# Boese0601/MagicDance

Hardware: NVIDIA H100
Metric: denoise-steps/sec @512x512 50-step DDIM (higher is better)
Workload: dtype f16

## Files before the change

### magicdance_b200/csrc/attention.cu

```cuda
#include <stdlib.h>

#include <type_traits>

#include "common.cuh"

namespace mdb {

constexpr int kBQ = 128;

template <int D, int BKV, int STAGES>
struct AttnCfg {
  static constexpr int kDkChunks = (D + 63) / 64;
  static constexpr int kDV = (D + 15) / 16 * 16;
  static constexpr int kKSteps = kDV / 16;
  static constexpr int kQBytes = kDkChunks * kBQ * 128;
  static constexpr int kKBytes = kDkChunks * BKV * 128;
  static constexpr int kVBytes = kDV * 128;
  static constexpr int kStageBytes = kKBytes + kVBytes;
  static constexpr int kSmem = kQBytes + STAGES * kStageBytes + 1024;
  static_assert(BKV == 64, "one 128-byte swizzle row of keys per V^T tile");
  static_assert(kVBytes % 1024 == 0 && kKBytes % 1024 == 0, "stage tiles start on swizzle-atom boundaries");
};

struct AttnKParams {
  CUtensorMap tmQ, tmK0, tmV0, tmK1, tmV1;
  __half* out;
  long long ldo;
  int nq, n0, n1;
  int kv0_batches, kv1_batches;
  int bank_batches;
  float scale_log2;
};
struct AttnLseKParams : AttnKParams {
  float* lse;
};

template <int D, int BKV, int STAGES, int MINB, bool LSE = false>
__global__ void __launch_bounds__(kWsThreads, MINB)
    attn_wg_kernel(const __grid_constant__ std::conditional_t<LSE, AttnLseKParams, AttnKParams> p) {
  using C = AttnCfg<D, BKV, STAGES>;
  extern __shared__ uint8_t smem_raw[];
  __shared__ __align__(8) uint64_t q_bar;
  __shared__ __align__(8) uint64_t kv_full[STAGES], kv_empty[STAGES];

  uint8_t* sQ = align1024(smem_raw);
  uint8_t* sKV = sQ + C::kQBytes;

  const int warp = threadIdx.x >> 5;
  const int lane = threadIdx.x & 31;
  const int q0 = blockIdx.x * kBQ;
  const int head = blockIdx.y;
  const int b = blockIdx.z;
  const int t0 = (p.n0 + BKV - 1) / BKV;
  const int t1 = (b < p.bank_batches && p.n1 > 0) ? (p.n1 + BKV - 1) / BKV : 0;
  const int n_tiles = t0 + t1;

  pdl_launch_dependents();
  if (warp == kProducerWarp && lane == 0) {
    tma_prefetch_desc(&p.tmQ);
    tma_prefetch_desc(&p.tmK0);
    tma_prefetch_desc(&p.tmV0);
    mbar_init(&q_bar, 1);
    ring_init<STAGES>(kv_full, kv_empty, 1);
    fence_barrier_init();
  }
  __syncthreads();
  pdl_wait();

  if (warp == kProducerWarp) {
    if (lane == 0) {
      mbar_expect_tx(&q_bar, C::kQBytes);
      for (int dc = 0; dc < C::kDkChunks; ++dc)
        tma_load_3d(sQ + dc * (kBQ * 128), &p.tmQ, &q_bar, dc * 64, head, b * p.nq + q0);
      for (int j = 0; j < n_tiles; ++j) {
        const bool src1 = j >= t0;
        const int key0 = (src1 ? (j - t0) : j) * BKV;
        const CUtensorMap* tk = src1 ? &p.tmK1 : &p.tmK0;
        const CUtensorMap* tv = src1 ? &p.tmV1 : &p.tmV0;
        const int nsrc = src1 ? p.n1 : p.n0;
        const int kvb = src1 ? (p.kv1_batches > 1 ? b : 0) : (p.kv0_batches > 1 ? b : 0);
        const int s = ring_acquire<STAGES>(kv_empty, j);
        mbar_expect_tx(&kv_full[s], C::kStageBytes);
        uint8_t* sk = sKV + s * C::kStageBytes;
        uint8_t* sv = sk + C::kKBytes;
        for (int dc = 0; dc < C::kDkChunks; ++dc)
          tma_load_3d(sk + dc * (BKV * 128), tk, &kv_full[s], dc * 64, head, kvb * nsrc + key0);
        tma_load_3d(sv, tv, &kv_full[s], key0, kvb, head * D);
      }
    }
  } else {
    const int wg = warp >> 2;
    const uint32_t q_addr = smem_u32(sQ) + wg * (64 * 128);
    const int cq = 2 * (lane & 3);
    float o[C::kDV / 2];
#pragma unroll
    for (int i = 0; i < C::kDV / 2; ++i) o[i] = 0.f;
    float m_run[2] = {-INFINITY, -INFINITY};
    float l_run[2] = {0.f, 0.f};
    mbar_wait(&q_bar, 0);

    for (int j = 0; j < n_tiles; ++j) {
      const bool src1 = j >= t0;
      const int key0 = (src1 ? (j - t0) : j) * BKV;
      const int valid = min(BKV, (src1 ? p.n1 : p.n0) - key0);
      const int s = ring_wait_full<STAGES>(kv_full, j);
      const uint32_t k_addr = smem_u32(sKV + s * C::kStageBytes);
      const uint32_t v_addr = k_addr + C::kKBytes;

      float sc[BKV / 2];
      wgmma_fence();
#pragma unroll
      for (int ks = 0; ks < C::kKSteps; ++ks) {
        const int dc = ks >> 2, kk = ks & 3;
        const uint64_t da = wgmma_desc_k_sw128(q_addr + dc * (kBQ * 128)) + 2 * kk;
        const uint64_t db = wgmma_desc_k_sw128(k_addr + dc * (BKV * 128)) + 2 * kk;
        wgmma_ss<BKV>(sc, da, db, ks != 0 ? 1u : 0u);
      }
      wgmma_commit();
      wgmma_wait<0>();
      wgmma_fence_regs(sc);

      if (valid < BKV) {
#pragma unroll
        for (int i = 0; i < BKV / 2; ++i)
          if (8 * (i >> 2) + cq + (i & 1) >= valid) sc[i] = -INFINITY;
      }
      float mx[2] = {-INFINITY, -INFINITY};
#pragma unroll
      for (int i = 0; i < BKV / 2; ++i) mx[(i >> 1) & 1] = fmaxf(mx[(i >> 1) & 1], sc[i]);
      float alpha[2], neg_m[2];
#pragma unroll
      for (int h = 0; h < 2; ++h) {
        mx[h] = fmaxf(mx[h], __shfl_xor_sync(0xffffffffu, mx[h], 1));
        mx[h] = fmaxf(mx[h], __shfl_xor_sync(0xffffffffu, mx[h], 2));
        const float m_new = fmaxf(m_run[h], mx[h] * p.scale_log2);
        alpha[h] = ex2_approx(m_run[h] - m_new);
        m_run[h] = m_new;
        neg_m[h] = -m_new;
      }
      float ls[2] = {0.f, 0.f};
      uint32_t pa[BKV / 16][4];
#pragma unroll
      for (int i = 0; i < BKV / 2; i += 2) {
        const int h = (i >> 1) & 1;
        const float e0 = ex2_approx(fmaf(sc[i], p.scale_log2, neg_m[h]));
        const float e1 = ex2_approx(fmaf(sc[i + 1], p.scale_log2, neg_m[h]));
        ls[h] += e0 + e1;
        pa[i >> 3][(i >> 1) & 3] = pack_half2(e0, e1);
      }
#pragma unroll
      for (int h = 0; h < 2; ++h) l_run[h] = fmaf(l_run[h], alpha[h], ls[h]);
#pragma unroll
      for (int i = 0; i < C::kDV / 2; ++i) o[i] *= alpha[(i >> 1) & 1];

      wgmma_fence();
#pragma unroll
      for (int kk = 0; kk < BKV / 16; ++kk)
        wgmma_rs<C::kDV>(o, pa[kk], wgmma_desc_k_sw128(v_addr) + 2 * kk, 1u);
      wgmma_commit();
      wgmma_wait<0>();
      wgmma_fence_regs(o);
      mbar_arrive(&kv_empty[s]);
    }

    float inv_l[2], l_row[2];
#pragma unroll
    for (int h = 0; h < 2; ++h) {
      float l = l_run[h];
      l += __shfl_xor_sync(0xffffffffu, l, 1);
      l += __shfl_xor_sync(0xffffffffu, l, 2);
      inv_l[h] = 1.0f / l;
      l_row[h] = l;
    }
    const int r = wg * 64 + (warp & 3) * 16 + (lane >> 2);
    if constexpr (LSE) {
      if ((lane & 3) == 0) {
#pragma unroll
        for (int h = 0; h < 2; ++h) {
          const int q = q0 + r + 8 * h;
          if (q < p.nq)
            p.lse[(static_cast<long long>(b) * gridDim.y + head) * p.nq + q] =
                (m_run[h] + log2f(l_row[h])) * 0.6931471805599453f;
        }
      }
    }
#pragma unroll
    for (int h = 0; h < 2; ++h) {
      const int q = q0 + r + 8 * h;
      if (q < p.nq) {
        __half* op = p.out + (static_cast<long long>(b) * p.nq + q) * p.ldo + head * D + cq;
#pragma unroll
        for (int c8 = 0; c8 < D / 8; ++c8)
          *reinterpret_cast<uint32_t*>(op + 8 * c8) =
              pack_half2(o[4 * c8 + 2 * h] * inv_l[h], o[4 * c8 + 2 * h + 1] * inv_l[h]);
      }
    }
  }
}

static int g_attn40_2q_min_ctas = 512;
int get_attn_tuning() { return g_attn40_2q_min_ctas; }
void set_attn_tuning(int v) { g_attn40_2q_min_ctas = v; }

template <int D, int BKV, int STAGES, int MINB, bool LSE = false, typename P>
static int launch_attn(const P& kp, dim3 grid, cudaStream_t st) {
  using C = AttnCfg<D, BKV, STAGES>;
  static_assert(MINB == 1 || C::kSmem <= 113 * 1024, "two CTAs per SM must fit");
  constexpr auto kern = attn_wg_kernel<D, BKV, STAGES, MINB, LSE>;
  if (int rc = set_max_dyn_smem<kern>(C::kSmem)) return rc;
  MDB_CHECK_CUDA(launch_pdl(kern, grid, dim3(kWsThreads), C::kSmem, st, kp));
  count_launch();
  return MDB_OK;
}

template <int D, int BKV>
static int build_and_launch(const mdb_attn_desc* a, float* lse, cudaStream_t st) {
  constexpr int kDV = AttnCfg<D, BKV, 1>::kDV;
  AttnKParams kp;
  memset(&kp, 0, sizeof(kp));
  const int hd = a->heads * a->d;
  int rc;
  if ((rc = tmap_heads(&kp.tmQ, a->q, a->d, a->heads, (uint64_t)a->batch * a->nq, a->ldq, kBQ))) return rc;
  auto mk_kv = [&](const void* k, long long ldk, const void* vt, long long ldvt, int n, int nb, int ldvb,
                   CUtensorMap* tk, CUtensorMap* tv) -> int {
    int r = tmap_heads(tk, k, a->d, a->heads, (uint64_t)nb * n, ldk, BKV);
    if (r) return r;
    return tmap_vt(tv, vt, n, nb, ldvb, hd, ldvt, kDV);
  };
  if ((rc = mk_kv(a->k0, a->ldk0, a->vt0, a->ldvt0, a->n0, a->kv0_batches, a->ldv0_batch, &kp.tmK0, &kp.tmV0))) return rc;
  if (a->n1 > 0) {
    if ((rc = mk_kv(a->k1, a->ldk1, a->vt1, a->ldvt1, a->n1, a->kv1_batches, a->ldv1_batch, &kp.tmK1, &kp.tmV1)))
      return rc;
  }
  kp.out = static_cast<__half*>(a->out);
  kp.ldo = a->ldo;
  kp.nq = a->nq;
  kp.n0 = a->n0;
  kp.n1 = a->n1;
  kp.kv0_batches = a->kv0_batches;
  kp.kv1_batches = a->kv1_batches;
  kp.bank_batches = a->n1 > 0 ? a->bank_batches : 0;
  kp.scale_log2 = a->scale * 1.4426950408889634f;
  dim3 grid((a->nq + kBQ - 1) / kBQ, a->heads, a->batch);
  if (lse != nullptr) {
    AttnLseKParams lp;
    memset(&lp, 0, sizeof(lp));
    static_cast<AttnKParams&>(lp) = kp;
    lp.lse = lse;
    if constexpr (D == 40) {
      const long long ctas = (long long)grid.x * grid.y * grid.z;
      if (ctas >= (long long)g_attn40_2q_min_ctas) return launch_attn<D, BKV, 3, 2, true>(lp, grid, st);
    }
    return launch_attn<D, BKV, (D == 160 ? 2 : 4), 1, true>(lp, grid, st);
  }
  if constexpr (D == 40) {
    const long long ctas = (long long)grid.x * grid.y * grid.z;
    if (ctas >= (long long)g_attn40_2q_min_ctas) return launch_attn<D, BKV, 3, 2>(kp, grid, st);
  }
  return launch_attn<D, BKV, (D == 160 ? 2 : 4), 1>(kp, grid, st);
}

static int attention_entry(const mdb_attn_desc* a, float* lse, cudaStream_t st) {
  switch (a->d) {
    case 40:
      return build_and_launch<40, 64>(a, lse, st);
    case 80:
      return build_and_launch<80, 64>(a, lse, st);
    case 160:
      return build_and_launch<160, 64>(a, lse, st);
    default:
      set_error("mdb_attention_f16: head dim %d not supported (40, 80, 160)", a->d);
      return MDB_ERR_UNSUPPORTED;
  }
}

int attention_check_desc(const mdb_attn_desc* a) {
  MDB_REQUIRE(a != nullptr, "mdb_attention_f16: null descriptor");
  MDB_REQUIRE(a->q && a->k0 && a->vt0 && a->out, "mdb_attention_f16: null operand");
  MDB_REQUIRE(a->batch > 0 && a->heads > 0 && a->nq > 0 && a->n0 > 0 && a->n1 >= 0,
              "mdb_attention_f16: bad shape");
  MDB_REQUIRE(a->n1 == 0 || (a->k1 && a->vt1), "mdb_attention_f16: n1 > 0 needs k1/vt1");
  MDB_REQUIRE(a->kv0_batches == 1 || a->kv0_batches == a->batch, "mdb_attention_f16: kv0_batches must be 1 or batch");
  MDB_REQUIRE(a->n1 == 0 || a->kv1_batches == 1 || a->kv1_batches >= a->bank_batches,
              "mdb_attention_f16: kv1_batches must be 1 or cover bank_batches");
  MDB_REQUIRE(a->ldv0_batch >= a->n0 && a->ldv0_batch % 8 == 0, "mdb_attention_f16: ldv0_batch must be >= n0 and %% 8");
  MDB_REQUIRE(a->n1 == 0 || (a->ldv1_batch >= a->n1 && a->ldv1_batch % 8 == 0),
              "mdb_attention_f16: ldv1_batch must be >= n1 and %% 8");
  MDB_REQUIRE(a->ldo % 8 == 0 && (reinterpret_cast<uintptr_t>(a->out) & 15) == 0, "mdb_attention_f16: out alignment");
  return MDB_OK;
}

}

using namespace mdb;

extern "C" int mdb_attention_f16(const mdb_attn_desc* a, mdb_stream_t stream) {
  const int rc = attention_check_desc(a);
  if (rc) return rc;
  return attention_entry(a, nullptr, static_cast<cudaStream_t>(stream));
}

extern "C" int mdb_attention_lse_f16(const mdb_attn_desc* a, float* lse, mdb_stream_t stream) {
  const int rc = attention_check_desc(a);
  if (rc) return rc;
  MDB_REQUIRE(lse != nullptr, "mdb_attention_lse_f16: null lse");
  return attention_entry(a, lse, static_cast<cudaStream_t>(stream));
}
```

### magicdance_b200/csrc/common.cuh

```cuda
#pragma once

#include <cuda.h>
#include <cuda_fp16.h>
#include <cuda_runtime.h>
#include <cudaTypedefs.h>
#include <stdint.h>
#include <stdio.h>
#include <string.h>

#include "../../include/magicdance_b200.h"
#include "wgmma.cuh"

namespace mdb {

void set_error(const char* fmt, ...);

#define MDB_CHECK_CUDA(expr)                                                                     \
  do {                                                                                           \
    cudaError_t _e = (expr);                                                                     \
    if (_e != cudaSuccess) {                                                                     \
      mdb::set_error("%s:%d: %s failed: %s", __FILE__, __LINE__, #expr, cudaGetErrorString(_e)); \
      return MDB_ERR_CUDA;                                                                       \
    }                                                                                            \
  } while (0)

#define MDB_REQUIRE(cond, ...)      \
  do {                              \
    if (!(cond)) {                  \
      mdb::set_error(__VA_ARGS__);  \
      return MDB_ERR_INVALID;       \
    }                               \
  } while (0)

void count_launch(int n = 1);
int get_gemm_tuning(int key);
void set_gemm_tuning(int key, int value);
int get_attn_tuning();
void set_attn_tuning(int v);

constexpr int kNumSms = 132;

int tmap_rows(CUtensorMap* out, const void* base, uint64_t inner, uint64_t rows, long long ld, uint32_t box_inner,
              uint32_t box_rows);
int tmap_heads(CUtensorMap* out, const void* base, int d, int heads, uint64_t tokens, long long ld,
               uint32_t box_tokens);
int tmap_heads_per_sample(CUtensorMap* out, const void* base, int d, int heads, int n, int nb, long long ld,
                          uint32_t box_tokens);
int tmap_vt(CUtensorMap* out, const void* base, int n, int nb, long long ldvb, int rows, long long ldvt,
            uint32_t box_rows);
int tmap_nhwc(CUtensorMap* out, const void* base, int c, int w, int h, int nb, long long ld, const uint32_t box[4],
              int cs);
int tmap_nhwc_im2col(CUtensorMap* out, const void* base, int c, int w, int h, int nb, long long ld, int pixels,
                     int cs);

enum { kBoxOk, kBoxWideRows, kBoxRowsPerTile, kBoxImagesPerTile, kBoxTooLarge };
int pixel_box(int ho, int wo, int cs, int rows, bool fwd, uint32_t box[4]);

#ifdef __CUDACC__

bool pdl_enabled();
template <typename... KArgs, typename... Args>
inline cudaError_t launch_pdl_cluster2(void (*kernel)(KArgs...), dim3 grid, dim3 block, size_t smem,
                                       cudaStream_t stream, unsigned cluster_x, unsigned cluster_z, Args&&... args) {
  cudaLaunchConfig_t cfg;
  memset(&cfg, 0, sizeof(cfg));
  cfg.gridDim = grid;
  cfg.blockDim = block;
  cfg.dynamicSmemBytes = smem;
  cfg.stream = stream;
  cudaLaunchAttribute attr[2];
  int n = 0;
  if (cluster_z > 1 || cluster_x > 1) {
    attr[n].id = cudaLaunchAttributeClusterDimension;
    attr[n].val.clusterDim.x = cluster_x;
    attr[n].val.clusterDim.y = 1;
    attr[n].val.clusterDim.z = cluster_z;
    ++n;
  }
  if (pdl_enabled()) {
    attr[n].id = cudaLaunchAttributeProgrammaticStreamSerialization;
    attr[n].val.programmaticStreamSerializationAllowed = 1;
    ++n;
  }
  cfg.attrs = attr;
  cfg.numAttrs = n;
  return cudaLaunchKernelEx(&cfg, kernel, static_cast<KArgs>(args)...);
}
template <typename... KArgs, typename... Args>
inline cudaError_t launch_pdl_cluster(void (*kernel)(KArgs...), dim3 grid, dim3 block, size_t smem,
                                      cudaStream_t stream, unsigned cluster_z, Args&&... args) {
  return launch_pdl_cluster2(kernel, grid, block, smem, stream, 1u, cluster_z, static_cast<Args&&>(args)...);
}
template <typename... KArgs, typename... Args>
inline cudaError_t launch_pdl(void (*kernel)(KArgs...), dim3 grid, dim3 block, size_t smem, cudaStream_t stream,
                              Args&&... args) {
  return launch_pdl_cluster2(kernel, grid, block, smem, stream, 1u, 1u, static_cast<Args&&>(args)...);
}
template <auto Kernel>
inline int set_max_dyn_smem(int bytes) {
  static bool done = false;
  if (!done) {
    MDB_CHECK_CUDA(cudaFuncSetAttribute(Kernel, cudaFuncAttributeMaxDynamicSharedMemorySize, bytes));
    done = true;
  }
  return MDB_OK;
}

__device__ __forceinline__ uint32_t smem_u32(const void* p) {
  return static_cast<uint32_t>(__cvta_generic_to_shared(p));
}

__device__ __forceinline__ bool elect_one() {
  uint32_t pred = 0;
  asm volatile(
      "{\n\t.reg .pred P;\n\t"
      "elect.sync _|P, 0xffffffff;\n\t"
      "selp.u32 %0, 1, 0, P;\n\t}"
      : "=r"(pred));
  return pred != 0;
}

__device__ __forceinline__ void pdl_launch_dependents() { asm volatile("griddepcontrol.launch_dependents;" ::: "memory"); }
__device__ __forceinline__ void pdl_wait() { asm volatile("griddepcontrol.wait;" ::: "memory"); }

__device__ __forceinline__ void mbar_init(uint64_t* bar, uint32_t count) {
  asm volatile("mbarrier.init.shared::cta.b64 [%0], %1;" ::"r"(smem_u32(bar)), "r"(count));
}
__device__ __forceinline__ void fence_barrier_init() {
  asm volatile("fence.mbarrier_init.release.cluster;" ::: "memory");
}
__device__ __forceinline__ void mbar_expect_tx(uint64_t* bar, uint32_t bytes) {
  asm volatile("mbarrier.arrive.expect_tx.shared::cta.b64 _, [%0], %1;" ::"r"(smem_u32(bar)), "r"(bytes)
               : "memory");
}
__device__ __forceinline__ void mbar_arrive(uint64_t* bar) {
  asm volatile("mbarrier.arrive.shared::cta.b64 _, [%0];" ::"r"(smem_u32(bar)) : "memory");
}
__device__ __forceinline__ void mbar_wait(uint64_t* bar, uint32_t parity) {
  uint32_t addr = smem_u32(bar);
  asm volatile(
      "{\n\t.reg .pred P1;\n\t"
      "WAIT_LOOP:\n\t"
      "mbarrier.try_wait.parity.shared::cta.b64 P1, [%0], %1;\n\t"
      "@P1 bra DONE;\n\t"
      "bra WAIT_LOOP;\n\t"
      "DONE:\n\t}"
      ::"r"(addr), "r"(parity)
      : "memory");
}

constexpr int kConsumers = 256;
constexpr int kProducerWarp = kConsumers / 32;
constexpr int kWsThreads = kConsumers + 32;

__device__ __forceinline__ uint8_t* align1024(uint8_t* p) {
  return reinterpret_cast<uint8_t*>((reinterpret_cast<uintptr_t>(p) + 1023) & ~uintptr_t(1023));
}

template <int S>
__device__ __forceinline__ void ring_init(uint64_t* full, uint64_t* empty, uint32_t full_count) {
  for (int s = 0; s < S; ++s) {
    mbar_init(&full[s], full_count);
    mbar_init(&empty[s], kConsumers);
  }
}
template <int S>
__device__ __forceinline__ int ring_acquire(uint64_t* empty, int it) {
  const int s = it % S;
  mbar_wait(&empty[s], ((it / S) & 1) ^ 1);
  return s;
}
template <int S>
__device__ __forceinline__ int ring_wait_full(uint64_t* full, int it) {
  const int s = it % S;
  mbar_wait(&full[s], (it / S) & 1);
  return s;
}

__device__ __forceinline__ void tma_prefetch_desc(const CUtensorMap* m) {
  asm volatile("prefetch.tensormap [%0];" ::"l"(reinterpret_cast<uint64_t>(m)) : "memory");
}
__device__ __forceinline__ void tma_load_2d(void* dst, const CUtensorMap* m, uint64_t* bar, int c0, int c1) {
  asm volatile(
      "cp.async.bulk.tensor.2d.shared::cluster.global.tile.mbarrier::complete_tx::bytes [%0], [%1, {%3, %4}], [%2];"
      ::"r"(smem_u32(dst)), "l"(reinterpret_cast<uint64_t>(m)), "r"(smem_u32(bar)), "r"(c0), "r"(c1)
      : "memory");
}
__device__ __forceinline__ void tma_load_3d(void* dst, const CUtensorMap* m, uint64_t* bar, int c0, int c1, int c2) {
  asm volatile(
      "cp.async.bulk.tensor.3d.shared::cluster.global.tile.mbarrier::complete_tx::bytes [%0], [%1, {%3, %4, %5}], [%2];"
      ::"r"(smem_u32(dst)), "l"(reinterpret_cast<uint64_t>(m)), "r"(smem_u32(bar)), "r"(c0), "r"(c1), "r"(c2)
      : "memory");
}
__device__ __forceinline__ void tma_load_4d(void* dst, const CUtensorMap* m, uint64_t* bar, int c0, int c1, int c2,
                                            int c3) {
  asm volatile(
      "cp.async.bulk.tensor.4d.shared::cluster.global.tile.mbarrier::complete_tx::bytes [%0], [%1, {%3, %4, %5, %6}], [%2];"
      ::"r"(smem_u32(dst)), "l"(reinterpret_cast<uint64_t>(m)), "r"(smem_u32(bar)), "r"(c0), "r"(c1), "r"(c2), "r"(c3)
      : "memory");
}
__device__ __forceinline__ void tma_load_im2col_4d(void* dst, const CUtensorMap* m, uint64_t* bar, int c0, int c1,
                                                   int c2, int c3, int ow, int oh) {
  const uint16_t w16 = static_cast<uint16_t>(ow), h16 = static_cast<uint16_t>(oh);
  asm volatile(
      "cp.async.bulk.tensor.4d.shared::cluster.global.im2col.mbarrier::complete_tx::bytes"
      " [%0], [%1, {%3, %4, %5, %6}], [%2], {%7, %8};"
      ::"r"(smem_u32(dst)), "l"(reinterpret_cast<uint64_t>(m)), "r"(smem_u32(bar)), "r"(c0), "r"(c1), "r"(c2), "r"(c3),
        "h"(w16), "h"(h16)
      : "memory");
}

__device__ __forceinline__ uint32_t cluster_ctarank() {
  uint32_t r;
  asm volatile("mov.u32 %0, %%cluster_ctarank;" : "=r"(r));
  return r;
}
__device__ __forceinline__ void cluster_sync_all() {
  asm volatile("barrier.cluster.arrive.release.aligned;" ::: "memory");
  asm volatile("barrier.cluster.wait.acquire.aligned;" ::: "memory");
}
__device__ __forceinline__ uint32_t dsmem_map(uint32_t local_smem_addr, uint32_t rank) {
  uint32_t a;
  asm volatile("mapa.shared::cluster.u32 %0, %1, %2;" : "=r"(a) : "r"(local_smem_addr), "r"(rank));
  return a;
}
__device__ __forceinline__ float4 dsmem_ld_f4(uint32_t cluster_addr) {
  float4 v;
  asm volatile("ld.shared::cluster.v4.f32 {%0, %1, %2, %3}, [%4];"
               : "=f"(v.x), "=f"(v.y), "=f"(v.z), "=f"(v.w)
               : "r"(cluster_addr));
  return v;
}

__device__ __forceinline__ void fence_proxy_async_smem() {
  asm volatile("fence.proxy.async.shared::cta;" ::: "memory");
}

__device__ __forceinline__ uint64_t wgmma_desc_k_sw128(uint32_t smem_addr) {
  uint64_t d = 0;
  d |= static_cast<uint64_t>((smem_addr & 0x3FFFF) >> 4);
  d |= static_cast<uint64_t>(1) << 16;
  d |= static_cast<uint64_t>(1024 >> 4) << 32;
  d |= static_cast<uint64_t>(1) << 62;
  return d;
}
__device__ __forceinline__ uint64_t wgmma_desc_mn_sw128(uint32_t smem_addr, uint32_t chunk_bytes) {
  uint64_t d = 0;
  d |= static_cast<uint64_t>((smem_addr & 0x3FFFF) >> 4);
  d |= static_cast<uint64_t>((chunk_bytes >> 4) & 0x3FFF) << 16;
  d |= static_cast<uint64_t>(1024 >> 4) << 32;
  d |= static_cast<uint64_t>(1) << 62;
  return d;
}
__device__ __forceinline__ void wgmma_fence() { asm volatile("wgmma.fence.sync.aligned;" ::: "memory"); }
__device__ __forceinline__ void wgmma_commit() { asm volatile("wgmma.commit_group.sync.aligned;" ::: "memory"); }
template <int N>
__device__ __forceinline__ void wgmma_wait() { asm volatile("wgmma.wait_group.sync.aligned %0;" ::"n"(N) : "memory"); }
template <int R>
__device__ __forceinline__ void wgmma_fence_regs(float (&d)[R]) {
#pragma unroll
  for (int i = 0; i < R; ++i) asm volatile("" : "+f"(d[i])::"memory");
}
__device__ __forceinline__ void named_bar_sync(int id, int threads) {
  asm volatile("bar.sync %0, %1;" ::"r"(id), "r"(threads) : "memory");
}

__device__ __forceinline__ uint32_t pack_half2(float a, float b) {
  __half2 h = __floats2half2_rn(a, b);
  return *reinterpret_cast<uint32_t*>(&h);
}

__device__ __forceinline__ float ex2_approx(float x) {
  float y;
  asm("ex2.approx.ftz.f32 %0, %1;" : "=f"(y) : "f"(x));
  return y;
}
__device__ __forceinline__ float silu_f(float x) { return x / (1.0f + __expf(-x)); }
__device__ __forceinline__ float gelu_erf_f(float x) { return 0.5f * x * (1.0f + erff(x * 0.70710678118654752f)); }
__device__ __forceinline__ float dsilu(float x) {
  const float s = 1.0f / (1.0f + __expf(-x));
  return s * (1.0f + x * (1.0f - s));
}
__device__ __forceinline__ float dgelu_erf(float x) {
  return 0.5f * (1.0f + erff(x * 0.70710678118654752f)) + x * 0.39894228040143268f * __expf(-0.5f * x * x);
}

struct GbOut {
  void* p;
  long long ld;
  int f32, acc;
};

__device__ __forceinline__ void gb_store2(const GbOut& o, long long row, int col, float v0, float v1) {
  if (o.p == nullptr) return;
  if (o.f32) {
    float2* d = reinterpret_cast<float2*>(static_cast<float*>(o.p) + row * o.ld + col);
    if (o.acc) {
      const float2 x = *d;
      v0 += x.x;
      v1 += x.y;
    }
    *d = make_float2(v0, v1);
  } else {
    __half2* d = reinterpret_cast<__half2*>(static_cast<__half*>(o.p) + row * o.ld + col);
    if (o.acc) {
      const float2 x = __half22float2(*d);
      v0 += x.x;
      v1 += x.y;
    }
    *d = __floats2half2_rn(v0, v1);
  }
}
#endif

inline GbOut gb_out(void* p, long long ld, int dtype, int acc) {
  GbOut o;
  o.p = p;
  o.ld = ld;
  o.f32 = dtype == MDB_DTYPE_F32;
  o.acc = acc != 0;
  return o;
}

int launch_colsum_finalize(const float* ws, int n, int segs, int parts, float* out, long long stride, int acc,
                           cudaStream_t st);

}
```

Baseline: 92.57.

## Pipeline attention QK^T with softmax and PV, add register rebalancing and 256-row Q tile

Reworks the warp-specialized flash-attention kernel so the QK^T wgmma for the next key tile is issued before the softmax of the current tile, using ping-pong score and probability buffers. A warpgroup-sized producer lowers its register budget with setmaxnreg while the consumers raise theirs. Every head dim now runs one CTA per SM with deeper stage counts. For d=40 on large grids, the old two-CTA-per-SM variant is replaced by a kernel that processes 256 query rows per CTA with four consumer warpgroups. The aim is to overlap tensor-core work with exponent math and cut K/V reloads, at the cost of more registers, a more complex wait-group schedule and lower CTA occupancy.

```diff
diff --git a/magicdance_b200/csrc/attention.cu b/magicdance_b200/csrc/attention.cu
--- a/magicdance_b200/csrc/attention.cu
+++ b/magicdance_b200/csrc/attention.cu
@@ -7,6 +7,10 @@
 namespace mdb {
 
 constexpr int kBQ = 128;
+constexpr int kAttnThreads = kConsumers + 128;
+constexpr int kAttnProducerRegs = 40;
+constexpr int kAttnConsumerRegs = 232;
+static_assert(128 * kAttnProducerRegs + kConsumers * kAttnConsumerRegs <= 65536, "the register file of one SM");
 
 template <int D, int BKV, int STAGES>
 struct AttnCfg {
@@ -20,6 +24,8 @@
   static constexpr int kSmem = kQBytes + STAGES * kStageBytes + 1024;
   static_assert(BKV == 64, "one 128-byte swizzle row of keys per V^T tile");
   static_assert(kVBytes % 1024 == 0 && kKBytes % 1024 == 0, "stage tiles start on swizzle-atom boundaries");
+  static_assert(kSmem <= 227 * 1024, "one CTA per SM");
+  static_assert(STAGES >= 3, "S(j + 1) is issued before stage j - 1 is released");
 };
 
 struct AttnKParams {
@@ -35,8 +41,16 @@
   float* lse;
 };
 
-template <int D, int BKV, int STAGES, int MINB, bool LSE = false>
-__global__ void __launch_bounds__(kWsThreads, MINB)
+template <int R>
+__device__ __forceinline__ void wgmma_fence_frags(uint32_t (&a)[R][4]) {
+#pragma unroll
+  for (int i = 0; i < R; ++i)
+#pragma unroll
+    for (int k = 0; k < 4; ++k) asm volatile("" : "+r"(a[i][k])::"memory");
+}
+
+template <int D, int BKV, int STAGES, bool LSE = false>
+__global__ void __launch_bounds__(kAttnThreads, 1)
     attn_wg_kernel(const __grid_constant__ std::conditional_t<LSE, AttnLseKParams, AttnKParams> p) {
   using C = AttnCfg<D, BKV, STAGES>;
   extern __shared__ uint8_t smem_raw[];
@@ -67,8 +81,9 @@
   __syncthreads();
   pdl_wait();
 
-  if (warp == kProducerWarp) {
-    if (lane == 0) {
+  if (warp >= kProducerWarp) {
+    setmaxnreg_dec<kAttnProducerRegs>();
+    if (warp == kProducerWarp && lane == 0) {
       mbar_expect_tx(&q_bar, C::kQBytes);
       for (int dc = 0; dc < C::kDkChunks; ++dc)
         tma_load_3d(sQ + dc * (kBQ * 128), &p.tmQ, &q_bar, dc * 64, head, b * p.nq + q0);
@@ -89,6 +104,214 @@
       }
     }
   } else {
+    setmaxnreg_inc<kAttnConsumerRegs>();
+    const int wg = warp >> 2;
+    const uint32_t q_addr = smem_u32(sQ) + wg * (64 * 128);
+    const int cq = 2 * (lane & 3);
+    float o[C::kDV / 2];
+#pragma unroll
+    for (int i = 0; i < C::kDV / 2; ++i) o[i] = 0.f;
+    float m_run[2] = {-INFINITY, -INFINITY};
+    float l_run[2] = {0.f, 0.f};
+    float s_a[BKV / 2], s_b[BKV / 2];
+    uint32_t p_a[BKV / 16][4], p_b[BKV / 16][4];
+    mbar_wait(&q_bar, 0);
+
+    auto issue_s = [&](float(&sc)[BKV / 2], int j) {
+      const int s = ring_wait_full<STAGES>(kv_full, j);
+      const uint32_t k_addr = smem_u32(sKV + s * C::kStageBytes);
+      wgmma_fence();
+#pragma unroll
+      for (int ks = 0; ks < C::kKSteps; ++ks) {
+        const int dc = ks >> 2, kk = ks & 3;
+        const uint64_t da = wgmma_desc_k_sw128(q_addr + dc * (kBQ * 128)) + 2 * kk;
+        const uint64_t db = wgmma_desc_k_sw128(k_addr + dc * (BKV * 128)) + 2 * kk;
+        wgmma_ss<BKV>(sc, da, db, ks != 0 ? 1u : 0u);
+      }
+      wgmma_commit();
+    };
+
+    auto step = [&](auto first, auto last, int j, float(&sc)[BKV / 2], float(&sn)[BKV / 2],
+                    uint32_t(&pc)[BKV / 16][4], uint32_t(&pp)[BKV / 16][4]) {
+      constexpr bool kFirst = decltype(first)::value, kLast = decltype(last)::value;
+      if constexpr (!kLast) issue_s(sn, j + 1);
+      wgmma_wait<int(!kFirst) + int(!kLast)>();
+      wgmma_fence_regs(sc);
+
+      const bool src1 = j >= t0;
+      const int key0 = (src1 ? (j - t0) : j) * BKV;
+      const int valid = min(BKV, (src1 ? p.n1 : p.n0) - key0);
+      if (valid < BKV) {
+#pragma unroll
+        for (int i = 0; i < BKV / 2; ++i)
+          if (8 * (i >> 2) + cq + (i & 1) >= valid) sc[i] = -INFINITY;
+      }
+      float mx[2] = {-INFINITY, -INFINITY};
+#pragma unroll
+      for (int i = 0; i < BKV / 2; ++i) mx[(i >> 1) & 1] = fmaxf(mx[(i >> 1) & 1], sc[i]);
+      float alpha[2], neg_m[2];
+#pragma unroll
+      for (int h = 0; h < 2; ++h) {
+        mx[h] = fmaxf(mx[h], __shfl_xor_sync(0xffffffffu, mx[h], 1));
+        mx[h] = fmaxf(mx[h], __shfl_xor_sync(0xffffffffu, mx[h], 2));
+        const float m_new = fmaxf(m_run[h], mx[h] * p.scale_log2);
+        alpha[h] = ex2_approx(m_run[h] - m_new);
+        m_run[h] = m_new;
+        neg_m[h] = -m_new;
+      }
+      float ls[2] = {0.f, 0.f};
+#pragma unroll
+      for (int i = 0; i < BKV / 2; i += 2) {
+        const int h = (i >> 1) & 1;
+        const float e0 = ex2_approx(fmaf(sc[i], p.scale_log2, neg_m[h]));
+        const float e1 = ex2_approx(fmaf(sc[i + 1], p.scale_log2, neg_m[h]));
+        ls[h] += e0 + e1;
+        pc[i >> 3][(i >> 1) & 3] = pack_half2(e0, e1);
+      }
+#pragma unroll
+      for (int h = 0; h < 2; ++h) l_run[h] = fmaf(l_run[h], alpha[h], ls[h]);
+
+      wgmma_fence_frags(pc);
+      wgmma_wait<int(!kLast)>();
+      wgmma_fence_regs(o);
+      if constexpr (!kFirst) {
+        wgmma_fence_frags(pp);
+        mbar_arrive(&kv_empty[(j - 1) % STAGES]);
+      }
+#pragma unroll
+      for (int i = 0; i < C::kDV / 2; ++i) o[i] *= alpha[(i >> 1) & 1];
+
+      const uint32_t v_addr = smem_u32(sKV + (j % STAGES) * C::kStageBytes) + C::kKBytes;
+      wgmma_fence();
+#pragma unroll
+      for (int kk = 0; kk < BKV / 16; ++kk)
+        wgmma_rs<C::kDV>(o, pc[kk], wgmma_desc_k_sw128(v_addr) + 2 * kk, 1u);
+      wgmma_commit();
+    };
+
+    using Yes = std::true_type;
+    using No = std::false_type;
+    issue_s(s_a, 0);
+    if (n_tiles == 1) {
+      step(Yes{}, Yes{}, 0, s_a, s_b, p_a, p_b);
+    } else {
+      step(Yes{}, No{}, 0, s_a, s_b, p_a, p_b);
+      int j = 1;
+      for (; j + 2 < n_tiles; j += 2) {
+        step(No{}, No{}, j, s_b, s_a, p_b, p_a);
+        step(No{}, No{}, j + 1, s_a, s_b, p_a, p_b);
+      }
+      if (j == n_tiles - 1) {
+        step(No{}, Yes{}, j, s_b, s_a, p_b, p_a);
+      } else {
+        step(No{}, No{}, j, s_b, s_a, p_b, p_a);
+        step(No{}, Yes{}, j + 1, s_a, s_b, p_a, p_b);
+      }
+    }
+    wgmma_wait<0>();
+    wgmma_fence_regs(o);
+    wgmma_fence_frags(p_a);
+    wgmma_fence_frags(p_b);
+    mbar_arrive(&kv_empty[(n_tiles - 1) % STAGES]);
+
+    float inv_l[2], l_row[2];
+#pragma unroll
+    for (int h = 0; h < 2; ++h) {
+      float l = l_run[h];
+      l += __shfl_xor_sync(0xffffffffu, l, 1);
+      l += __shfl_xor_sync(0xffffffffu, l, 2);
+      inv_l[h] = 1.0f / l;
+      l_row[h] = l;
+    }
+    const int r = wg * 64 + (warp & 3) * 16 + (lane >> 2);
+    if constexpr (LSE) {
+      if ((lane & 3) == 0) {
+#pragma unroll
+        for (int h = 0; h < 2; ++h) {
+          const int q = q0 + r + 8 * h;
+          if (q < p.nq)
+            p.lse[(static_cast<long long>(b) * gridDim.y + head) * p.nq + q] =
+                (m_run[h] + log2f(l_row[h])) * 0.6931471805599453f;
+        }
+      }
+    }
+#pragma unroll
+    for (int h = 0; h < 2; ++h) {
+      const int q = q0 + r + 8 * h;
+      if (q < p.nq) {
+        __half* op = p.out + (static_cast<long long>(b) * p.nq + q) * p.ldo + head * D + cq;
+#pragma unroll
+        for (int c8 = 0; c8 < D / 8; ++c8)
+          *reinterpret_cast<uint32_t*>(op + 8 * c8) =
+              pack_half2(o[4 * c8 + 2 * h] * inv_l[h], o[4 * c8 + 2 * h + 1] * inv_l[h]);
+      }
+    }
+  }
+}
+
+constexpr int kQ256Threads = 4 * 128 + 32;
+template <int D, int BKV, int STAGES, bool LSE = false>
+__global__ void __launch_bounds__(kQ256Threads, 1)
+    attn_wg_kernel_q256(const __grid_constant__ std::conditional_t<LSE, AttnLseKParams, AttnKParams> p) {
+  using C = AttnCfg<D, BKV, STAGES>;
+  extern __shared__ uint8_t smem_raw[];
+  __shared__ __align__(8) uint64_t q_bar;
+  __shared__ __align__(8) uint64_t kv_full[STAGES], kv_empty[STAGES];
+
+  constexpr int BQ = 256;
+  constexpr int kQBytes = C::kDkChunks * BQ * 128;
+  constexpr int kProd = 16;
+  uint8_t* sQ = align1024(smem_raw);
+  uint8_t* sKV = sQ + kQBytes;
+
+  const int warp = threadIdx.x >> 5;
+  const int lane = threadIdx.x & 31;
+  const int q0 = blockIdx.x * BQ;
+  const int head = blockIdx.y;
+  const int b = blockIdx.z;
+  const int t0 = (p.n0 + BKV - 1) / BKV;
+  const int t1 = (b < p.bank_batches && p.n1 > 0) ? (p.n1 + BKV - 1) / BKV : 0;
+  const int n_tiles = t0 + t1;
+
+  pdl_launch_dependents();
+  if (warp == kProd && lane == 0) {
+    tma_prefetch_desc(&p.tmQ);
+    tma_prefetch_desc(&p.tmK0);
+    tma_prefetch_desc(&p.tmV0);
+    mbar_init(&q_bar, 1);
+    for (int st = 0; st < STAGES; ++st) {
+      mbar_init(&kv_full[st], 1);
+      mbar_init(&kv_empty[st], 4 * 128);
+    }
+    fence_barrier_init();
+  }
+  __syncthreads();
+  pdl_wait();
+
+  if (warp == kProd) {
+    if (lane == 0) {
+      mbar_expect_tx(&q_bar, kQBytes);
+      for (int dc = 0; dc < C::kDkChunks; ++dc)
+        for (int hq = 0; hq < BQ / kBQ; ++hq)
+          tma_load_3d(sQ + dc * (BQ * 128) + hq * (kBQ * 128), &p.tmQ, &q_bar, dc * 64, head,
+                      b * p.nq + q0 + hq * kBQ);
+      for (int j = 0; j < n_tiles; ++j) {
+        const bool src1 = j >= t0;
+        const int key0 = (src1 ? (j - t0) : j) * BKV;
+        const CUtensorMap* tk = src1 ? &p.tmK1 : &p.tmK0;
+        const CUtensorMap* tv = src1 ? &p.tmV1 : &p.tmV0;
+        const int nsrc = src1 ? p.n1 : p.n0;
+        const int kvb = src1 ? (p.kv1_batches > 1 ? b : 0) : (p.kv0_batches > 1 ? b : 0);
+        const int s = ring_acquire<STAGES>(kv_empty, j);
+        mbar_expect_tx(&kv_full[s], C::kStageBytes);
+        uint8_t* sk = sKV + s * C::kStageBytes;
+        uint8_t* sv = sk + C::kKBytes;
+        for (int dc = 0; dc < C::kDkChunks; ++dc)
+          tma_load_3d(sk + dc * (BKV * 128), tk, &kv_full[s], dc * 64, head, kvb * nsrc + key0);
+        tma_load_3d(sv, tv, &kv_full[s], key0, kvb, head * D);
+      }
+    }
+  } else {
     const int wg = warp >> 2;
     const uint32_t q_addr = smem_u32(sQ) + wg * (64 * 128);
     const int cq = 2 * (lane & 3);
@@ -112,7 +335,7 @@
 #pragma unroll
       for (int ks = 0; ks < C::kKSteps; ++ks) {
         const int dc = ks >> 2, kk = ks & 3;
-        const uint64_t da = wgmma_desc_k_sw128(q_addr + dc * (kBQ * 128)) + 2 * kk;
+        const uint64_t da = wgmma_desc_k_sw128(q_addr + dc * (BQ * 128)) + 2 * kk;
         const uint64_t db = wgmma_desc_k_sw128(k_addr + dc * (BKV * 128)) + 2 * kk;
         wgmma_ss<BKV>(sc, da, db, ks != 0 ? 1u : 0u);
       }
@@ -198,24 +421,43 @@
   }
 }
 
+template <int D>
+struct AttnPlan {
+  static constexpr int kBKV = 64;
+  static constexpr int kStages = D == 160 ? 3 : 4;
+};
+
+template <int D, bool LSE, typename P>
+static int launch_attn(const P& kp, dim3 grid, cudaStream_t st) {
+  using Plan = AttnPlan<D>;
+  using C = AttnCfg<D, Plan::kBKV, Plan::kStages>;
+  constexpr auto kern = attn_wg_kernel<D, Plan::kBKV, Plan::kStages, LSE>;
+  if (int rc = set_max_dyn_smem<kern>(C::kSmem)) return rc;
+  MDB_CHECK_CUDA(launch_pdl(kern, grid, dim3(kAttnThreads), C::kSmem, st, kp));
+  count_launch();
+  return MDB_OK;
+}
+template <bool LSE, typename P>
+static int launch_attn40_q256(const P& kp, dim3 grid, cudaStream_t st) {
+  using C = AttnCfg<40, 64, 6>;
+  constexpr int kSmem = C::kSmem + C::kQBytes;
+  static_assert(kSmem <= 227 * 1024, "one CTA per SM");
+  constexpr auto kern = attn_wg_kernel_q256<40, 64, 6, LSE>;
+  if (int rc = set_max_dyn_smem<kern>(kSmem)) return rc;
+  grid.x = (grid.x + 1) / 2;
+  MDB_CHECK_CUDA(launch_pdl(kern, grid, dim3(kQ256Threads), kSmem, st, kp));
+  count_launch();
+  return MDB_OK;
+}
+
 static int g_attn40_2q_min_ctas = 512;
 int get_attn_tuning() { return g_attn40_2q_min_ctas; }
 void set_attn_tuning(int v) { g_attn40_2q_min_ctas = v; }
 
-template <int D, int BKV, int STAGES, int MINB, bool LSE = false, typename P>
-static int launch_attn(const P& kp, dim3 grid, cudaStream_t st) {
-  using C = AttnCfg<D, BKV, STAGES>;
-  static_assert(MINB == 1 || C::kSmem <= 113 * 1024, "two CTAs per SM must fit");
-  constexpr auto kern = attn_wg_kernel<D, BKV, STAGES, MINB, LSE>;
-  if (int rc = set_max_dyn_smem<kern>(C::kSmem)) return rc;
-  MDB_CHECK_CUDA(launch_pdl(kern, grid, dim3(kWsThreads), C::kSmem, st, kp));
-  count_launch();
-  return MDB_OK;
-}
-
-template <int D, int BKV>
+template <int D>
 static int build_and_launch(const mdb_attn_desc* a, float* lse, cudaStream_t st) {
-  constexpr int kDV = AttnCfg<D, BKV, 1>::kDV;
+  constexpr int BKV = AttnPlan<D>::kBKV;
+  constexpr int kDV = AttnCfg<D, BKV, AttnPlan<D>::kStages>::kDV;
   AttnKParams kp;
   memset(&kp, 0, sizeof(kp));
   const int hd = a->heads * a->d;
@@ -242,32 +484,29 @@
   kp.bank_batches = a->n1 > 0 ? a->bank_batches : 0;
   kp.scale_log2 = a->scale * 1.4426950408889634f;
   dim3 grid((a->nq + kBQ - 1) / kBQ, a->heads, a->batch);
+  const long long ctas = (long long)grid.x * grid.y * grid.z;
   if (lse != nullptr) {
     AttnLseKParams lp;
     memset(&lp, 0, sizeof(lp));
     static_cast<AttnKParams&>(lp) = kp;
     lp.lse = lse;
-    if constexpr (D == 40) {
-      const long long ctas = (long long)grid.x * grid.y * grid.z;
-      if (ctas >= (long long)g_attn40_2q_min_ctas) return launch_attn<D, BKV, 3, 2, true>(lp, grid, st);
-    }
-    return launch_attn<D, BKV, (D == 160 ? 2 : 4), 1, true>(lp, grid, st);
-  }
-  if constexpr (D == 40) {
-    const long long ctas = (long long)grid.x * grid.y * grid.z;
-    if (ctas >= (long long)g_attn40_2q_min_ctas) return launch_attn<D, BKV, 3, 2>(kp, grid, st);
-  }
-  return launch_attn<D, BKV, (D == 160 ? 2 : 4), 1>(kp, grid, st);
+    if constexpr (D == 40)
+      if (ctas >= (long long)g_attn40_2q_min_ctas) return launch_attn40_q256<true>(lp, grid, st);
+    return launch_attn<D, true>(lp, grid, st);
+  }
+  if constexpr (D == 40)
+    if (ctas >= (long long)g_attn40_2q_min_ctas) return launch_attn40_q256<false>(kp, grid, st);
+  return launch_attn<D, false>(kp, grid, st);
 }
 
 static int attention_entry(const mdb_attn_desc* a, float* lse, cudaStream_t st) {
   switch (a->d) {
     case 40:
-      return build_and_launch<40, 64>(a, lse, st);
+      return build_and_launch<40>(a, lse, st);
     case 80:
-      return build_and_launch<80, 64>(a, lse, st);
+      return build_and_launch<80>(a, lse, st);
     case 160:
-      return build_and_launch<160, 64>(a, lse, st);
+      return build_and_launch<160>(a, lse, st);
     default:
       set_error("mdb_attention_f16: head dim %d not supported (40, 80, 160)", a->d);
       return MDB_ERR_UNSUPPORTED;
diff --git a/magicdance_b200/csrc/common.cuh b/magicdance_b200/csrc/common.cuh
--- a/magicdance_b200/csrc/common.cuh
+++ b/magicdance_b200/csrc/common.cuh
@@ -261,6 +261,10 @@
 #pragma unroll
   for (int i = 0; i < R; ++i) asm volatile("" : "+f"(d[i])::"memory");
 }
+template <int R>
+__device__ __forceinline__ void setmaxnreg_dec() { asm volatile("setmaxnreg.dec.sync.aligned.u32 %0;" ::"n"(R)); }
+template <int R>
+__device__ __forceinline__ void setmaxnreg_inc() { asm volatile("setmaxnreg.inc.sync.aligned.u32 %0;" ::"n"(R)); }
 __device__ __forceinline__ void named_bar_sync(int id, int threads) {
   asm volatile("bar.sync %0, %1;" ::"r"(id), "r"(threads) : "memory");
 }
```

Result: no change. 93.01, median of 6 (+0.5%).
